# facebookresearch/PhysicsVAE

Measured on AMD Instinct MI355X. Metric: train samples/sec (world-model+VAE step), loco demo, batch 256, 1/2/4/8 GPU, higher is better.
Workload: dtype f32; 1 GPU; BASELINE configs[1-2]: synthetic loco demo 10x1000, dim_state_body 197, dim_action 45, batch 256/GPU, TE/MD/WM 4x1024, joint phase; phase=joint, global_batch=256, parallelism=dp1, first_layers=staged

## Files before the change

physicsvae_amd/csrc/pvae_gemm_fused.h:

```cpp
#pragma once
#include "pvae_gemm_common.h"
#include "pvae_stage.h"
#include "pvae_gemm_src.h"
#include "pvae_gemm_reg.h"
#include "pvae_gemm_wgrad.h"
#include "pvae_adam.h"

namespace pvae {
template <class Epi, int ABL = 0>
__global__ void __launch_bounds__(256)
gemm_wgrad_reg_kernel(PVAE_GA_PARAMS(a_), int nw, Epi epi, AdamPair ad) {
    const GemmArgs ga = PVAE_GA_OF(a_);
    __shared__ __attribute__((aligned(16))) float lds[kPairLdsFloats];
    const int b = blockIdx.x, nb = bias_tiles(ga);
    if (b < nw) wgrad_body<Epi, ABL>(lds, b, ga, epi);
    else if (b < nw + nb) bias_grad_body(lds, b - nw, ga, epi);
    else adam_pair_body(ad, b - nw - nb);
}

struct TouchRuns {
    const float* p[4];
    int lines[4];
    int blocks;
};
__device__ inline void touch_body(const TouchRuns& t, int blk) {
    float sink = 0.f;
#pragma unroll
    for (int r = 0; r < 4; ++r)
        for (int i = blk * 256 + (int)threadIdx.x; i < t.lines[r]; i += t.blocks * 256)
            asm volatile("global_load_dword %0, %1, off" : "+v"(sink) : "v"(t.p[r] + (size_t)i * 32) : "memory");
    asm volatile("s_waitcnt vmcnt(0)" : "+v"(sink)::"memory");
}
template <class EpiW>
__global__ void __launch_bounds__(256, 3)
wgrad_pair_gather_kernel(const float* aQ, const float* g_s0, const float* g_s1, unsigned a_ld, unsigned a_t, unsigned a_k,
                         unsigned g_ld0n0, unsigned g_ld1n1, unsigned g_rq1, int g_b0, int g_b1, int na, EpiW e1, AdamPair ad,
                         TouchRuns touch, XSrc rest) {
    __shared__ __attribute__((aligned(16))) float lds[kPairLdsFloats];
    GemmArgs g1 = ga_unpack(aQ, nullptr, a_ld, a_t, a_k);
    const int gfl = g1.krot;
    g1.krot = 0;
    PGather ps;
    ps.x = rest;
    ps.x.s0 = g_s0; ps.x.ld0 = (int)(g_ld0n0 & 0xffffu); ps.x.n0 = (int)(g_ld0n0 >> 16);
    ps.x.s1 = g_s1; ps.x.ld1 = (int)(g_ld1n1 & 0xffffu); ps.x.n1 = (int)(g_ld1n1 >> 16);
    ps.x.ind1 = (gfl >> 1) & 1;
    ps.x.rows = (int)(g_rq1 & 0xffffu) + 1;
    ps.x.rm.seg = gfl & 1; ps.x.rm.q1 = (int)(g_rq1 >> 16) + 1; ps.x.rm.b0 = g_b0; ps.x.rm.b1 = g_b1;
    const int n1 = ga_grid(g1), nb1 = bias_tiles(g1);
    const int b = blockIdx.x;
    if (b < n1) wgrad_body<EpiW, 0, PGather>(lds, b, g1, e1, ps);
    else if (b < n1 + nb1) bias_grad_body(lds, b - n1, g1, e1);
    else if (b < n1 + nb1 + na) adam_pair_body(ad, b - n1 - nb1);
    else touch_body(touch, b - n1 - nb1 - na);
}
template <class EpiD, class EpiW, class PS>
__global__ void __launch_bounds__(256, 3)
bwd_pair_gather_kernel(PVAE_GA2_PARAMS, EpiD ed, EpiW ew, AdamPair ad, PS ps) {
    __shared__ __attribute__((aligned(16))) float lds[kPairLdsFloats];
    const GemmArgs gd = PVAE_GA2_A, gw = PVAE_GA2_B;
    const int nd = ga_grid(gd), nw = ga_grid(gw);
    const int b = blockIdx.x;
    if (b < nd) {
        if (gd.tile16) splitk_reg16_body<false, EpiD>(lds, b, gd, ed);
        else splitk_reg_body<false, EpiD, 0>(lds, b, gd, ed);
    } else if (b < nd + nw) wgrad_body<EpiW, 0, PS>(lds, b - nd, gw, ew, ps);
    else if (b < nd + nw + bias_tiles(gw)) bias_grad_body(lds, b - nd - nw, gw, ew);
    else adam_pair_body(ad, b - nd - nw - bias_tiles(gw));
}

template <class EpiW>
__global__ void __launch_bounds__(256)
wgrad_pair_kernel(PVAE_GA2_PARAMS, int na, EpiW e1, EpiW e2, StageArgs sa, AdamPair ad) {
    __shared__ __attribute__((aligned(16))) float lds[kPairLdsFloats];
    const GemmArgs g1 = PVAE_GA2_A, g2 = PVAE_GA2_B;
    const int n1 = ga_grid(g1), n12 = n1 + ga_grid(g2);
    const int b = blockIdx.x;
    const int nb1 = bias_tiles(g1), nb2 = bias_tiles(g2);
    if (b < n1) wgrad_body<EpiW>(lds, b, g1, e1);
    else if (b < n12) wgrad_body<EpiW>(lds, b - n1, g2, e2);
    else if (b < n12 + nb1) bias_grad_body(lds, b - n12, g1, e1);
    else if (b < n12 + nb1 + nb2) bias_grad_body(lds, b - n12 - nb1, g2, e2);
    else if (b < n12 + nb1 + nb2 + na) adam_pair_body(ad, b - n12 - nb1 - nb2);
    else stage_row(sa, b - n12 - nb1 - nb2 - na, 0, sa.rows_pad);
}

template <class EpiD, class EpiW, int ABL = 0>
__global__ void __launch_bounds__(256)
bwd_pair_kernel(PVAE_GA2_PARAMS, EpiD ed, EpiW ew, AdamPair ad) {
    __shared__ __attribute__((aligned(16))) float lds[kPairLdsFloats];
    const GemmArgs gd = PVAE_GA2_A, gw = PVAE_GA2_B;
    const int nd = ga_grid(gd), nw = ga_grid(gw);
    PVAE_MARK(0, 0);
    PVAE_MARK_HW();
    const int b = blockIdx.x;
    if (b < nd) {
        if (gd.tile16) splitk_reg16_body<false, EpiD>(lds, b, gd, ed);
        else splitk_reg_body<false, EpiD, ABL>(lds, b, gd, ed);
    } else if (b < nd + nw) wgrad_body<EpiW, ABL>(lds, b - nd, gw, ew);
    else if (b < nd + nw + bias_tiles(gw)) bias_grad_body(lds, b - nd - nw, gw, ew);
    else adam_pair_body(ad, b - nd - nw - bias_tiles(gw));
    PVAE_MARK(0, 3);
}

template <class EpiD, class EpiW>
__global__ void __launch_bounds__(256)
bwd_pair64_kernel(PVAE_GA2_PARAMS, EpiD ed, EpiW ew, AdamPair ad) {
    __shared__ __attribute__((aligned(16))) float lds[kReg64RingFloats];
    const GemmArgs gd = PVAE_GA2_A, gw = PVAE_GA2_B;
    const int nd = ga_grid(gd), nw = ga_grid(gw);
    const int b = blockIdx.x;
    if (b < nd) splitk_reg64_body<EpiD>(lds, b, gd, ed);
    else if (b < nd + nw) wgrad_body<EpiW>(lds, b - nd, gw, ew);
    else if (b < nd + nw + bias_tiles(gw)) bias_grad_body(lds, b - nd - nw, gw, ew);
    else adam_pair_body(ad, b - nd - nw - bias_tiles(gw));
}
}
```

physicsvae_amd/csrc/pvae_gemm_reg.h:

```cpp
#pragma once
#include "pvae_gemm_common.h"

namespace pvae {
template <bool P_ROW>
__device__ inline void store_partial_32x32(float* red, const v4f (&acc)[2][2], int li, int lh) {
    constexpr int RS = 36;
#pragma unroll
    for (int a = 0; a < 2; ++a) {
        float* row = red + (16 * a + li) * RS;
        if (P_ROW) {
#pragma unroll
            for (int b = 0; b < 2; ++b) *reinterpret_cast<v4f*>(row + 16 * b + 4 * lh) = acc[a][b];
        } else {
            *reinterpret_cast<v4f*>(row + 8 * lh) = v4f{acc[a][0][0], acc[a][1][0], acc[a][0][1], acc[a][1][1]};
            *reinterpret_cast<v4f*>(row + 8 * lh + 4) = v4f{acc[a][0][2], acc[a][1][2], acc[a][0][3], acc[a][1][3]};
        }
    }
}

template <bool P_ROW, class Epi, int ABL = 0>
__device__ inline void splitk_reg_body(float* lds, int bid, const GemmArgs& ga, Epi& epi) {
    constexpr int BK = 64, kTile = 32 * 64, kStage = 2 * kTile, D = kRegDepthD, S = 2;
    static_assert(S * kStage >= 4 * 32 * 36, "ring must hold the split-K reduction buffer");
    const float* __restrict__ Q = ga.Q;
    const float* __restrict__ P = ga.P;
    const int ldq = ga.ldq, ldp = ga.ldp, K = ga.K, tiles_q = ga.tiles_q, tiles_p = ga.tiles_p;

    const int xcd = bid & 7, loc = bid >> 3;
    const int tile_p = xcd * ga.p_per_xcd + loc / tiles_q;
    const int tile_q = loc % tiles_q;
    if (tile_p >= tiles_p) return;
    const int q0 = tile_q * 32, p0 = tile_p * 32;

    const int tid = threadIdx.x;
    const int lane = tid & 63;
    const int wave = tid >> 6;
    const int li = lane & 15, lh = lane >> 4;

    const float* sq[2];
    const float* sp[2];
    int slot_off[2];
#pragma unroll
    for (int u = 0; u < 2; ++u) {
        const int j = (wave + 4 * u) * 64 + lane;
        slot_off[u] = j * 4;
        {
            const int row = j >> 4, c = (j & 15) ^ (row & 15);
            sq[u] = Q + (size_t)(q0 + row) * ldq + c * 4;
        }
        if (P_ROW) {
            const int row = j >> 4, c = (j & 15) ^ (row & 15);
            sp[u] = P + (size_t)(p0 + row) * ldp + c * 4;
        } else {
            const int r = j >> 3, k = r ^ ((r >> 2) & 1);
            sp[u] = P + (size_t)k * ldp + p0 + (j & 7) * 4;
        }
    }
    const size_t kstep_p = P_ROW ? (size_t)BK : (size_t)BK * ldp;

    v4f rg[D][4];
    auto gload = [&](int t, v4f(&r)[4]) {
        r[0] = *reinterpret_cast<const v4f*>(sq[0] + (size_t)t * BK);
        r[1] = *reinterpret_cast<const v4f*>(sp[0] + (size_t)t * kstep_p);
        r[2] = *reinterpret_cast<const v4f*>(sq[1] + (size_t)t * BK);
        r[3] = *reinterpret_cast<const v4f*>(sp[1] + (size_t)t * kstep_p);
    };
    auto lwrite = [&](float* slot, const v4f(&r)[4]) {
        *reinterpret_cast<v4f*>(slot + slot_off[0]) = r[0];
        *reinterpret_cast<v4f*>(slot + kTile + slot_off[0]) = r[1];
        *reinterpret_cast<v4f*>(slot + slot_off[1]) = r[2];
        *reinterpret_cast<v4f*>(slot + kTile + slot_off[1]) = r[3];
    };

    v4f acc[2][2];
#pragma unroll
    for (int a = 0; a < 2; ++a)
#pragma unroll
        for (int b = 0; b < 2; ++b) acc[a][b] = v4f{0.f, 0.f, 0.f, 0.f};

    int oq[2];
#pragma unroll
    for (int a = 0; a < 2; ++a) {
        const int row = 16 * a + li;
        oq[a] = row * 64 + (((4 * wave + lh) ^ (row & 15)) << 2);
    }
    const int kq = 16 * wave + 4 * lh;

    const int nk = K / BK;
#pragma unroll
    for (int d = 0; d < D; ++d) gload(d < nk ? d : nk - 1, rg[d]);
    lwrite(lds, rg[0]);
    gload(D < nk ? D : nk - 1, rg[0]);
    const typename Epi::Pre epre = epi.preload(q0 + (tid >> 3), p0 + ((tid & 7) << 2));
    __syncthreads();

    v4f abl_q = v4f{1.f, 2.f, 3.f, 4.f} * (float)(lane + 1);
    asm volatile("" : "+v"(abl_q));
    auto tile_step = [&](int t, int d, bool guarded) {
        const float* st = lds + (t & 1) * kStage;
        v4f fq[2], fp[2];
        v2f fc[4];
        if (ABL & 2) {
#pragma unroll
            for (int a = 0; a < 2; ++a) { fq[a] = abl_q; fp[a] = abl_q; }
#pragma unroll
            for (int s2 = 0; s2 < 4; ++s2) fc[s2] = v2f{abl_q[0], abl_q[1]};
            asm volatile("" : "+v"(fq[0]), "+v"(fq[1]), "+v"(fp[0]), "+v"(fp[1]));
        } else {
#pragma unroll
            for (int a = 0; a < 2; ++a) fq[a] = *reinterpret_cast<const v4f*>(st + oq[a]);
            if (P_ROW) {
#pragma unroll
                for (int b = 0; b < 2; ++b) fp[b] = *reinterpret_cast<const v4f*>(st + kTile + oq[b]);
            } else {
#pragma unroll
                for (int s2 = 0; s2 < 4; ++s2)
                    fc[s2] = *reinterpret_cast<const v2f*>(st + kTile + (((kq + s2) ^ (lh & 1)) * 32) + 2 * li);
            }
        }
#pragma unroll
        for (int s2 = 0; s2 < 4; ++s2) {
#pragma unroll
            for (int a = 0; a < 2; ++a)
#pragma unroll
                for (int b = 0; b < 2; ++b) {
                    const float pv = P_ROW ? fp[b][s2] : fc[s2][b];
                    if (ABL & 4) acc[a][b][0] += pv * fq[a][s2];
                    else acc[a][b] = __builtin_amdgcn_mfma_f32_16x16x4f32(pv, fq[a][s2], acc[a][b], 0, 0, 0);
                }
            if (s2 == 1 && !(ABL & 1)) {
                if (!guarded) {
                    lwrite(lds + ((t + 1) & 1) * kStage, rg[(d + 1) % D]);
                    const int tn = t + 1 + D < nk ? t + 1 + D : nk - 1;
                    gload(tn, rg[(d + 1) % D]);
                } else if (t + 1 < nk) {
                    lwrite(lds + ((t + 1) & 1) * kStage, rg[(d + 1) % D]);
                    if (t + 1 + D < nk) gload(t + 1 + D, rg[(d + 1) % D]);
                }
            }
        }
        if (!(ABL & 8)) __syncthreads();
    };
    int t0 = 0;
    for (; t0 + D <= nk; t0 += D) {
#pragma unroll
        for (int d = 0; d < D; ++d) tile_step(t0 + d, d, false);
    }
#pragma unroll
    for (int d = 0; d < D; ++d)
        if (t0 + d < nk) tile_step(t0 + d, d, true);

    constexpr int RS = 36;
    store_partial_32x32<P_ROW>(lds + wave * (32 * RS), acc, li, lh);
    __syncthreads();
    {
        const int ql = tid >> 3, pl = (tid & 7) << 2;
        v4f v = *reinterpret_cast<const v4f*>(lds + ql * RS + pl);
#pragma unroll
        for (int w = 1; w < 4; ++w) v += *reinterpret_cast<const v4f*>(lds + w * (32 * RS) + ql * RS + pl);
        epi(q0 + ql, p0 + pl, v, epre);
    }
    epi.finish(lds, tile_q * tiles_p + tile_p, tid);
}


constexpr int kReg64RingFloats = 2 * (64 * 64 + 64 * 32);
template <class Epi>
__device__ inline void splitk_reg64_body(float* lds, int bid, const GemmArgs& ga, Epi& epi) {
    constexpr int BK = 64, kTileQ = 64 * 64, kTileP = 64 * 32, kStage = kTileQ + kTileP, D = kRegDepthD64;
    constexpr int RS = 36;
    static_assert(2 * kStage >= 4 * 64 * RS, "ring must hold the split-K reduction buffer");
    const float* __restrict__ Q = ga.Q;
    const float* __restrict__ P = ga.P;
    const int ldq = ga.ldq, ldp = ga.ldp, K = ga.K, tiles_q = ga.tiles_q, tiles_p = ga.tiles_p;
    const int xcd = bid & 7, loc = bid >> 3;
    const int tile_p = xcd * ga.p_per_xcd + loc / tiles_q;
    const int tile_q = loc % tiles_q;
    if (tile_p >= tiles_p) return;
    const int q0 = tile_q * 64, p0 = tile_p * 32;
    const int tid = threadIdx.x, lane = tid & 63, wave = tid >> 6;
    const int li = lane & 15, lh = lane >> 4;

    const float* sq[4];
    const float* sp[2];
#pragma unroll
    for (int u = 0; u < 4; ++u) {
        const int j = tid + 256 * u, row = j >> 4, c = (j & 15) ^ (row & 15);
        sq[u] = Q + (size_t)(q0 + row) * ldq + c * 4;
    }
#pragma unroll
    for (int u = 0; u < 2; ++u) {
        const int j = tid + 256 * u, r = j >> 3, k = r ^ ((r >> 2) & 1);
        sp[u] = P + (size_t)k * ldp + p0 + (j & 7) * 4;
    }
    const size_t kstep_p = (size_t)BK * ldp;
    v4f rg[D][6];
    auto gload = [&](int t, v4f(&r)[6]) {
#pragma unroll
        for (int u = 0; u < 4; ++u) r[u] = *reinterpret_cast<const v4f*>(sq[u] + (size_t)t * BK);
#pragma unroll
        for (int u = 0; u < 2; ++u) r[4 + u] = *reinterpret_cast<const v4f*>(sp[u] + (size_t)t * kstep_p);
    };
    auto lwrite = [&](float* slot, const v4f(&r)[6]) {
#pragma unroll
        for (int u = 0; u < 4; ++u) *reinterpret_cast<v4f*>(slot + (tid + 256 * u) * 4) = r[u];
#pragma unroll
        for (int u = 0; u < 2; ++u) *reinterpret_cast<v4f*>(slot + kTileQ + (tid + 256 * u) * 4) = r[4 + u];
    };
    v4f acc[4][2];
#pragma unroll
    for (int a = 0; a < 4; ++a)
#pragma unroll
        for (int b = 0; b < 2; ++b) acc[a][b] = v4f{0.f, 0.f, 0.f, 0.f};
    int oq[4];
#pragma unroll
    for (int a = 0; a < 4; ++a) {
        const int row = 16 * a + li;
        oq[a] = row * 64 + (((4 * wave + lh) ^ (row & 15)) << 2);
    }
    const int kq = 16 * wave + 4 * lh;
    const int nk = K / BK;
#pragma unroll
    for (int d = 0; d < D; ++d) gload(d < nk ? d : nk - 1, rg[d]);
    lwrite(lds, rg[0]);
    gload(D < nk ? D : nk - 1, rg[0]);
    typename Epi::Pre epre[2];
#pragma unroll
    for (int h = 0; h < 2; ++h) epre[h] = epi.preload(q0 + 32 * h + (tid >> 3), p0 + ((tid & 7) << 2));
    __syncthreads();
    auto tile_step = [&](int t, int d, bool guarded) {
        const float* st = lds + (t & 1) * kStage;
        v4f fq[4];
        v2f fc[4];
#pragma unroll
        for (int a = 0; a < 4; ++a) fq[a] = *reinterpret_cast<const v4f*>(st + oq[a]);
#pragma unroll
        for (int s2 = 0; s2 < 4; ++s2)
            fc[s2] = *reinterpret_cast<const v2f*>(st + kTileQ + (((kq + s2) ^ (lh & 1)) * 32) + 2 * li);
#pragma unroll
        for (int s2 = 0; s2 < 4; ++s2) {
#pragma unroll
            for (int a = 0; a < 4; ++a)
#pragma unroll
                for (int b = 0; b < 2; ++b)
                    acc[a][b] = __builtin_amdgcn_mfma_f32_16x16x4f32(fc[s2][b], fq[a][s2], acc[a][b], 0, 0, 0);
            if (s2 == 1) {
                if (!guarded) {
                    lwrite(lds + ((t + 1) & 1) * kStage, rg[(d + 1) % D]);
                    const int tn = t + 1 + D < nk ? t + 1 + D : nk - 1;
                    gload(tn, rg[(d + 1) % D]);
                } else if (t + 1 < nk) {
                    lwrite(lds + ((t + 1) & 1) * kStage, rg[(d + 1) % D]);
                    if (t + 1 + D < nk) gload(t + 1 + D, rg[(d + 1) % D]);
                }
            }
        }
        __syncthreads();
    };
    int t0 = 0;
    for (; t0 + D <= nk; t0 += D) {
#pragma unroll
        for (int d = 0; d < D; ++d) tile_step(t0 + d, d, false);
    }
#pragma unroll
    for (int d = 0; d < D; ++d)
        if (t0 + d < nk) tile_step(t0 + d, d, true);

    float* red = lds + wave * (64 * RS);
#pragma unroll
    for (int a = 0; a < 4; ++a) {
        float* row = red + (16 * a + li) * RS;
        *reinterpret_cast<v4f*>(row + 8 * lh) = v4f{acc[a][0][0], acc[a][1][0], acc[a][0][1], acc[a][1][1]};
        *reinterpret_cast<v4f*>(row + 8 * lh + 4) = v4f{acc[a][0][2], acc[a][1][2], acc[a][0][3], acc[a][1][3]};
    }
    __syncthreads();
#pragma unroll
    for (int h = 0; h < 2; ++h) {
        const int ql = 32 * h + (tid >> 3), pl = (tid & 7) << 2;
        v4f v = *reinterpret_cast<const v4f*>(lds + ql * RS + pl);
#pragma unroll
        for (int w = 1; w < 4; ++w) v += *reinterpret_cast<const v4f*>(lds + w * (64 * RS) + ql * RS + pl);
        epi(q0 + ql, p0 + pl, v, epre[h]);
    }
    epi.finish(lds, tile_q * tiles_p + tile_p, tid);
}

template <bool P_ROW, class Epi, int ABL = 0>
__global__ void __launch_bounds__(256)
gemm_splitk_reg_kernel(PVAE_GA_PARAMS(a_), Epi epi) {
    const GemmArgs ga = PVAE_GA_OF(a_);
    __shared__ __attribute__((aligned(16))) float lds[kRegRingFloats];
    splitk_reg_body<P_ROW, Epi, ABL>(lds, blockIdx.x, ga, epi);
}

template <bool P_ROW, class Epi>
__device__ inline void splitk_reg16_body(float* lds, int bid, const GemmArgs& ga, Epi& epi) {
    constexpr int BK = 64, kTile = 16 * 64, kStage = 2 * kTile, D = kRegDepth16;
    const float* __restrict__ Q = ga.Q;
    const float* __restrict__ P = ga.P;
    const int ldq = ga.ldq, ldp = ga.ldp, K = ga.K, tiles_q = ga.tiles_q, tiles_p = ga.tiles_p;

    const int xcd = bid & 7, loc = bid >> 3;
    const int tile_p = xcd * ga.p_per_xcd + loc / tiles_q;
    const int tile_q = loc % tiles_q;
    if (tile_p >= tiles_p) return;
    const int q0 = tile_q * 16, p0 = tile_p * 16;

    const int tid = threadIdx.x;
    const int lane = tid & 63;
    const int wave = tid >> 6;
    const int li = lane & 15, lh = lane >> 4;

    const int srow = tid >> 4, schunk = (tid & 15) ^ srow;
    const float* sq = Q + (size_t)(q0 + srow) * ldq + schunk * 4;
    const float* sp = P_ROW ? P + (size_t)(p0 + srow) * ldp + schunk * 4
                            : P + (size_t)(tid >> 2) * ldp + p0 + (tid & 3) * 4;
    const size_t kstep_p = P_ROW ? (size_t)BK : (size_t)BK * ldp;
    const int slot_off = tid * 4;
    const int pk = tid >> 2;
    const int slot_off_p = P_ROW ? slot_off : ((pk ^ ((pk >> 2) & 1)) * 16 + (tid & 3) * 4);

    v4f rg[D][2];
    auto gload = [&](int t, v4f(&r)[2]) {
        r[0] = *reinterpret_cast<const v4f*>(sq + (size_t)t * BK);
        r[1] = *reinterpret_cast<const v4f*>(sp + (size_t)t * kstep_p);
    };
    auto lwrite = [&](float* slot, const v4f(&r)[2]) {
        *reinterpret_cast<v4f*>(slot + slot_off) = r[0];
        *reinterpret_cast<v4f*>(slot + kTile + slot_off_p) = r[1];
    };
    v4f acc[2] = {v4f{0.f, 0.f, 0.f, 0.f}, v4f{0.f, 0.f, 0.f, 0.f}};
    const int of = li * 64 + (((4 * wave + lh) ^ li) << 2);

    const int nk = K / BK;
#pragma unroll
    for (int d = 0; d < D; ++d) gload(d < nk ? d : nk - 1, rg[d]);
    lwrite(lds, rg[0]);
    gload(D < nk ? D : nk - 1, rg[0]);
    __syncthreads();

    auto tile_step = [&](int t, int d, bool guarded) {
        const float* st = lds + (t & 1) * kStage;
        const v4f fq = *reinterpret_cast<const v4f*>(st + of);
        v4f fp;
        if (P_ROW) {
            fp = *reinterpret_cast<const v4f*>(st + kTile + of);
        } else {
#pragma unroll
            for (int s2 = 0; s2 < 4; ++s2) fp[s2] = st[kTile + ((16 * wave + 4 * lh + s2) ^ (lh & 1)) * 16 + li];
        }
#pragma unroll
        for (int s2 = 0; s2 < 4; ++s2) {
            acc[s2 & 1] = __builtin_amdgcn_mfma_f32_16x16x4f32(fp[s2], fq[s2], acc[s2 & 1], 0, 0, 0);
            if (s2 == 1) {
                if (!guarded) {
                    lwrite(lds + ((t + 1) & 1) * kStage, rg[(d + 1) % D]);
                    const int tn = t + 1 + D < nk ? t + 1 + D : nk - 1;
                    gload(tn, rg[(d + 1) % D]);
                } else if (t + 1 < nk) {
                    lwrite(lds + ((t + 1) & 1) * kStage, rg[(d + 1) % D]);
                    if (t + 1 + D < nk) gload(t + 1 + D, rg[(d + 1) % D]);
                }
            }
        }
        __syncthreads();
    };
    int t0 = 0;
    for (; t0 + D <= nk; t0 += D) {
#pragma unroll
        for (int d = 0; d < D; ++d) tile_step(t0 + d, d, false);
    }
#pragma unroll
    for (int d = 0; d < D; ++d)
        if (t0 + d < nk) tile_step(t0 + d, d, true);

    constexpr int RS = 20;
    float* red = lds + wave * (16 * RS);
    const v4f mine = acc[0] + acc[1];
    *reinterpret_cast<v4f*>(red + li * RS + 4 * lh) = mine;
    __syncthreads();
    if (tid < 64) {
        const int ql = tid >> 2, pl = (tid & 3) << 2;
        v4f v = *reinterpret_cast<const v4f*>(lds + ql * RS + pl);
#pragma unroll
        for (int w = 1; w < 4; ++w) v += *reinterpret_cast<const v4f*>(lds + w * (16 * RS) + ql * RS + pl);
        epi(q0 + ql, p0 + pl, v, epi.preload(q0 + ql, p0 + pl));
    }
    epi.finish(lds, tile_q * tiles_p + tile_p, tid);
}

template <bool P_ROW, class Epi>
__global__ void __launch_bounds__(256)
gemm_splitk_reg16_kernel(PVAE_GA_PARAMS(a_), Epi epi) {
    const GemmArgs ga = PVAE_GA_OF(a_);
    __shared__ __attribute__((aligned(16))) float lds[2 * 2 * 16 * 64];
    splitk_reg16_body<P_ROW, Epi>(lds, blockIdx.x, ga, epi);
}
}
```

Baseline: 1.148 million samples/s.

## Make split-K staging wave-private to replace block barriers with wave-level ordering

Remaps how each thread stages Q/P tiles into LDS so that every wave writes exactly the K-chunk slice that it later reads as MFMA fragments. This lets the per-tile __syncthreads in the split-K register GEMM bodies become a wavefront fence plus wave barrier, with one block barrier kept before the cross-wave reduction. The intent is to remove inter-wave stalls in the K loop. The change depends on the new staging layout exactly matching each wave's fragment reads for both P_ROW and column-P paths, and wgrad is excluded from one ABL variant. A layout mismatch would cause silent data races.

```diff
diff --git a/physicsvae_amd/csrc/pvae_gemm_fused.h b/physicsvae_amd/csrc/pvae_gemm_fused.h
--- a/physicsvae_amd/csrc/pvae_gemm_fused.h
+++ b/physicsvae_amd/csrc/pvae_gemm_fused.h
@@ -97,7 +97,7 @@
     if (b < nd) {
         if (gd.tile16) splitk_reg16_body<false, EpiD>(lds, b, gd, ed);
         else splitk_reg_body<false, EpiD, ABL>(lds, b, gd, ed);
-    } else if (b < nd + nw) wgrad_body<EpiW, ABL>(lds, b - nd, gw, ew);
+    } else if (b < nd + nw) wgrad_body<EpiW, (ABL & 32) ? 0 : ABL>(lds, b - nd, gw, ew);
     else if (b < nd + nw + bias_tiles(gw)) bias_grad_body(lds, b - nd - nw, gw, ew);
     else adam_pair_body(ad, b - nd - nw - bias_tiles(gw));
     PVAE_MARK(0, 3);
diff --git a/physicsvae_amd/csrc/pvae_gemm_reg.h b/physicsvae_amd/csrc/pvae_gemm_reg.h
--- a/physicsvae_amd/csrc/pvae_gemm_reg.h
+++ b/physicsvae_amd/csrc/pvae_gemm_reg.h
@@ -2,6 +2,15 @@
 #include "pvae_gemm_common.h"
 
 namespace pvae {
+__device__ inline int stage_row16(int lane) {
+    const int m = lane >> 2;
+    return (m & 8) | ((m & 1) << 2) | ((m >> 1) & 3);
+}
+__device__ inline void wave_order_point() {
+    __builtin_amdgcn_fence(__ATOMIC_RELEASE, "wavefront");
+    __builtin_amdgcn_wave_barrier();
+    __builtin_amdgcn_fence(__ATOMIC_ACQUIRE, "wavefront");
+}
 template <bool P_ROW>
 __device__ inline void store_partial_32x32(float* red, const v4f (&acc)[2][2], int li, int lh) {
     constexpr int RS = 36;
@@ -39,21 +48,19 @@
 
     const float* sq[2];
     const float* sp[2];
-    int slot_off[2];
+    int slot_off[2], slot_off_p[2];
 #pragma unroll
     for (int u = 0; u < 2; ++u) {
-        const int j = (wave + 4 * u) * 64 + lane;
-        slot_off[u] = j * 4;
-        {
-            const int row = j >> 4, c = (j & 15) ^ (row & 15);
-            sq[u] = Q + (size_t)(q0 + row) * ldq + c * 4;
-        }
+        const int row = 16 * u + stage_row16(lane), c = 4 * wave + (lane & 3);
+        slot_off[u] = (row * 16 + (c ^ (row & 15))) * 4;
+        sq[u] = Q + (size_t)(q0 + row) * ldq + c * 4;
         if (P_ROW) {
-            const int row = j >> 4, c = (j & 15) ^ (row & 15);
+            slot_off_p[u] = slot_off[u];
             sp[u] = P + (size_t)(p0 + row) * ldp + c * 4;
         } else {
-            const int r = j >> 3, k = r ^ ((r >> 2) & 1);
-            sp[u] = P + (size_t)k * ldp + p0 + (j & 7) * 4;
+            const int k = 16 * wave + 8 * u + (lane >> 3);
+            slot_off_p[u] = (k ^ ((k >> 2) & 1)) * 32 + (lane & 7) * 4;
+            sp[u] = P + (size_t)k * ldp + p0 + (lane & 7) * 4;
         }
     }
     const size_t kstep_p = P_ROW ? (size_t)BK : (size_t)BK * ldp;
@@ -67,9 +74,9 @@
     };
     auto lwrite = [&](float* slot, const v4f(&r)[4]) {
         *reinterpret_cast<v4f*>(slot + slot_off[0]) = r[0];
-        *reinterpret_cast<v4f*>(slot + kTile + slot_off[0]) = r[1];
+        *reinterpret_cast<v4f*>(slot + kTile + slot_off_p[0]) = r[1];
         *reinterpret_cast<v4f*>(slot + slot_off[1]) = r[2];
-        *reinterpret_cast<v4f*>(slot + kTile + slot_off[1]) = r[3];
+        *reinterpret_cast<v4f*>(slot + kTile + slot_off_p[1]) = r[3];
     };
 
     v4f acc[2][2];
@@ -92,7 +99,7 @@
     lwrite(lds, rg[0]);
     gload(D < nk ? D : nk - 1, rg[0]);
     const typename Epi::Pre epre = epi.preload(q0 + (tid >> 3), p0 + ((tid & 7) << 2));
-    __syncthreads();
+    wave_order_point();
 
     v4f abl_q = v4f{1.f, 2.f, 3.f, 4.f} * (float)(lane + 1);
     asm volatile("" : "+v"(abl_q));
@@ -139,7 +146,7 @@
                 }
             }
         }
-        if (!(ABL & 8)) __syncthreads();
+        if (!(ABL & 8)) wave_order_point();
     };
     int t0 = 0;
     for (; t0 + D <= nk; t0 += D) {
@@ -150,6 +157,7 @@
     for (int d = 0; d < D; ++d)
         if (t0 + d < nk) tile_step(t0 + d, d, true);
 
+    __syncthreads();
     constexpr int RS = 36;
     store_partial_32x32<P_ROW>(lds + wave * (32 * RS), acc, li, lh);
     __syncthreads();
@@ -311,12 +319,12 @@
     const int wave = tid >> 6;
     const int li = lane & 15, lh = lane >> 4;
 
-    const int srow = tid >> 4, schunk = (tid & 15) ^ srow;
+    const int srow = stage_row16(lane), schunk = 4 * wave + (lane & 3);
     const float* sq = Q + (size_t)(q0 + srow) * ldq + schunk * 4;
     const float* sp = P_ROW ? P + (size_t)(p0 + srow) * ldp + schunk * 4
                             : P + (size_t)(tid >> 2) * ldp + p0 + (tid & 3) * 4;
     const size_t kstep_p = P_ROW ? (size_t)BK : (size_t)BK * ldp;
-    const int slot_off = tid * 4;
+    const int slot_off = (srow * 16 + (schunk ^ srow)) * 4;
     const int pk = tid >> 2;
     const int slot_off_p = P_ROW ? slot_off : ((pk ^ ((pk >> 2) & 1)) * 16 + (tid & 3) * 4);
 
@@ -337,18 +345,20 @@
     for (int d = 0; d < D; ++d) gload(d < nk ? d : nk - 1, rg[d]);
     lwrite(lds, rg[0]);
     gload(D < nk ? D : nk - 1, rg[0]);
-    __syncthreads();
-
-    auto tile_step = [&](int t, int d, bool guarded) {
-        const float* st = lds + (t & 1) * kStage;
-        const v4f fq = *reinterpret_cast<const v4f*>(st + of);
-        v4f fp;
+    wave_order_point();
+
+    auto frag_read = [&](const float* st, v4f& fq, v4f& fp) {
+        fq = *reinterpret_cast<const v4f*>(st + of);
         if (P_ROW) {
             fp = *reinterpret_cast<const v4f*>(st + kTile + of);
         } else {
 #pragma unroll
             for (int s2 = 0; s2 < 4; ++s2) fp[s2] = st[kTile + ((16 * wave + 4 * lh + s2) ^ (lh & 1)) * 16 + li];
         }
+    };
+    auto tile_step = [&](int t, int d, bool guarded) {
+        v4f fq, fp;
+        frag_read(lds + (t & 1) * kStage, fq, fp);
 #pragma unroll
         for (int s2 = 0; s2 < 4; ++s2) {
             acc[s2 & 1] = __builtin_amdgcn_mfma_f32_16x16x4f32(fp[s2], fq[s2], acc[s2 & 1], 0, 0, 0);
@@ -363,7 +373,7 @@
                 }
             }
         }
-        __syncthreads();
+        wave_order_point();
     };
     int t0 = 0;
     for (; t0 + D <= nk; t0 += D) {
@@ -374,6 +384,7 @@
     for (int d = 0; d < D; ++d)
         if (t0 + d < nk) tile_step(t0 + d, d, true);
 
+    __syncthreads();
     constexpr int RS = 20;
     float* red = lds + wave * (16 * RS);
     const v4f mine = acc[0] + acc[1];
```

Result: faster. 1.164 million samples/s, median of 6 (+1.4%).
